# Rongjiehuang/FastDiff

Hardware: AMD Instinct MI355X
Metric: real-time factor (audio-sec/wall-sec), N=4 reverse steps, 80x864 mel (higher is better)
Workload: dtype f32 results; 2-piece fp16 operands (22 bit) on fp16 MFMA, fp32 accumulate; GEMM as Winograd F(2,3); exact-fp32 twin; 1 GPU; BASELINE configs[1]: LJSpeech shape, batch=8 x 80x864 mel per GPU, N=4, HIP kernels + hipGraph sampler; batch_per_gpu=8, frames=864, reverse_steps=4, graph=True, weights=random init seed 1234 (no checkpoint offline), world_size=1, gpus_visible=1, oversubscribed=False

## Files before the change

fastdiff_amd/csrc/fd_kernels_lvc.hip:

```cpp
#include "fd_kernels_common.h"

namespace fdk_fast {

template <int HOP, int DIL>
struct LvcCfg {
    static constexpr int WC = 64;
    static constexpr int W = 4 * WC;
    static constexpr int H = (DIL + 1 + 3) & ~3;
    static constexpr int XLD = W + 2 * H;
    static constexpr int YLD = W + 4;
};

#ifdef FD_LVC_TIMING
__device__ long long fd_dbg[64 * 4 * 8];
#define FD_STAMP(i) do { if (lane == 0 && blockIdx.y == FD_LVC_TIMING && blockIdx.x >= 100 && blockIdx.x < 164) \
        fd_dbg[((blockIdx.x - 100) * 4 + wave) * 8 + (i)] = (long long)__builtin_amdgcn_s_memtime(); } while (0)
#elif defined(FD_LVC_TIMELINE)
__device__ long long *fd_tl;
#define FD_STAMP_AT(i) do { if (threadIdx.x == 0) { long long *q_ = fd_tl + ((size_t)blockIdx.y * gridDim.x + blockIdx.x) * 10; \
        q_[i] = (long long)__builtin_amdgcn_s_memrealtime(); \
        if ((i) == 0) { q_[8] = __builtin_amdgcn_s_getreg(63492); q_[9] = __builtin_amdgcn_s_getreg(63508); } } } while (0)
#if defined(FD_TL_VARIANT)
#define FD_STAMP(i) do { if ((i) == 0 || (i) == 6 || (i) == 7) FD_STAMP_AT(i); else if ((i) == 1) FD_STAMP_AT(5); } while (0)
#define FD_STAMP_X(i) FD_STAMP_AT(i)
#else
#define FD_STAMP(i) FD_STAMP_AT(i)
#endif
#else
#define FD_STAMP(i)
#endif
#ifndef FD_STAMP_X
#define FD_STAMP_X(i)
#endif

__device__ __forceinline__ float gate(float a, float b)
{
    typedef float f2 __attribute__((ext_vector_type(2)));
    b = fmaxf(b, -15.0f);
    const f2 e = f2{a, b} * f2{-1.4426950408889634f, -2.8853900817779268f};
    const f2 uv = f2{__builtin_amdgcn_exp2f(e.x), __builtin_amdgcn_exp2f(e.y)};
    const f2 d = uv + 1.0f;
    return (1.0f - uv.y) * __builtin_amdgcn_rcpf(d.x * d.y);
}

template <int HOP, int DIL>
__global__ void __launch_bounds__(256, 2) k_lvc_layer(const float *__restrict__ xin, const float *__restrict__ skip,
                                                      float *__restrict__ xout, const float *__restrict__ kpack, int layer,
                                                      const float *__restrict__ wpack, const float *__restrict__ wref,
                                                      const float *__restrict__ cbias, int T, const int *__restrict__ run_if,
                                                      const int *__restrict__ lens)
{
    static_assert(HOP >= 64, "hop 8 has its own kernel (k_lvc_h8)");
    using Cfg = LvcCfg<HOP, DIL>;
    if (run_if && *run_if == 0) return;
    constexpr int WC = Cfg::WC, W = Cfg::W, H = Cfg::H, XLD = Cfg::XLD, YLD = Cfg::YLD, NT = WC / 32;
    constexpr int LT = (HOP == 256) ? 1 : 2;
    constexpr int LN = (HOP == 256) ? 4 : 2;
    constexpr bool PREACT = (HOP == 256);
    __shared__ __attribute__((aligned(16))) float xs[fd::C * XLD];
    __shared__ __attribute__((aligned(16))) float ys[fd::C * YLD];
    const int Ln = T * HOP;
    const int b = blockIdx.y, w0 = blockIdx.x * W;
    const int Tb = frames_of(lens, b, T), Lnb = Tb * HOP;
    if (w0 >= Lnb) return;
    const int tid = threadIdx.x, lane = tid & 63, wave = tid >> 6, l31 = lane & 31, hi = lane >> 5;
    const int cw = wave * WC;
    const bool wave_valid = (w0 + cw) < Lnb;
    const int mt0 = (HOP == 256) ? (wave & 1) : 0;
    const int lcw = (HOP == 256) ? 128 * (wave >> 1) : cw;
    FD_STAMP(0);

    float4 ka[LT][12];
    float4 bz[LT][4];
    if constexpr (HOP >= 64) {
        if (wave_valid) {
            const int f = (w0 + lcw) / HOP;
            const float *rec = kpack + ((int64_t)b * T + f) * fd::KREC;
            const float4 *kp4 = reinterpret_cast<const float4 *>(rec + layer * fd::KLAYER) + 2 * lane;
            const float4 *kb4 = reinterpret_cast<const float4 *>(rec + fd::KW + layer * 64);
#pragma unroll
            for (int m = 0; m < LT; ++m) {
#pragma unroll
                for (int i = 0; i < 12; ++i) ka[m][i] = kp4[((mt0 + m) * 6 + (i >> 1)) * 128 + (i & 1)];
#pragma unroll
                for (int j = 0; j < 4; ++j) bz[m][j] = kb4[(mt0 + m) * 8 + 2 * j + hi];
            }
        }
    }
    float4 wa[12];
#pragma unroll
    for (int i = 0; i < 12; ++i) wa[i] = reinterpret_cast<const float4 *>(wpack)[i * 64 + lane];
    float4 cb[4];
#pragma unroll
    for (int j = 0; j < 4; ++j) cb[j] = reinterpret_cast<const float4 *>(cbias)[2 * j + hi];
    {
        const float *xr = xin + (int64_t)b * fd::C * Ln, *sr = skip + (int64_t)b * fd::C * Ln;
        constexpr int NF4 = XLD / 4, TOTAL = fd::C * NF4, NK = (TOTAL + 255) / 256;
        constexpr int NB = (HOP == 64) ? 2 : 1, KB = (NK + NB - 1) / NB;
#pragma unroll
        for (int bt = 0; bt < NB; ++bt) {
            float4 xa[KB], sa[KB];
#pragma unroll
            for (int k = 0; k < KB; ++k) {
                const int idx = (bt * KB + k) * 256 + tid, ci = idx / NF4, c4 = idx - ci * NF4, g = w0 - H + 4 * c4;
                const bool ok = idx < TOTAL && g >= 0 && g < Lnb;
                xa[k] = ok ? *reinterpret_cast<const float4 *>(xr + (int64_t)ci * Ln + g) : make_float4(0.f, 0.f, 0.f, 0.f);
                sa[k] = ok ? *reinterpret_cast<const float4 *>(sr + (int64_t)ci * Ln + g) : make_float4(0.f, 0.f, 0.f, 0.f);
            }
            __builtin_amdgcn_sched_barrier(0);
#pragma unroll
            for (int k = 0; k < KB; ++k) {
                const int idx = (bt * KB + k) * 256 + tid, ci = idx / NF4, c4 = idx - ci * NF4;
                if (idx < TOTAL) {
                    const float4 r = make_float4(xa[k].x + sa[k].x, xa[k].y + sa[k].y, xa[k].z + sa[k].z, xa[k].w + sa[k].w);
                    if constexpr (PREACT) {
                        *reinterpret_cast<float4 *>(xs + ci * XLD + 4 * c4) =
                            make_float4(lrelu(r.x, 0.2f), lrelu(r.y, 0.2f), lrelu(r.z, 0.2f), lrelu(r.w, 0.2f));
                        if (c4 >= H / 4 && c4 < H / 4 + W / 4) *reinterpret_cast<float4 *>(ys + ci * YLD + 4 * c4 - H) = r;
                    } else {
                        *reinterpret_cast<float4 *>(xs + ci * XLD + 4 * c4) = r;
                    }
                }
            }
        }
    }
    const int hside = tid >> 7, ho = (tid & 127) >> 2, hq = tid & 3;
    __syncthreads();
    FD_STAMP(1);
    float resid[PREACT ? LN : 1][PREACT ? 8 * LT : 1];
    if constexpr (PREACT) {
#pragma unroll
        for (int nt = 0; nt < LN; ++nt)
#pragma unroll
            for (int m = 0; m < LT; ++m)
#pragma unroll
                for (int r = 0; r < 8; ++r)
                    resid[nt][m * 8 + r] = ys[(16 * (mt0 + m) + (r & 3) + 8 * (r >> 2) + 4 * hi) * YLD + lcw + nt * 32 + l31];
        __syncthreads();
    }

    if (wave_valid) {
        f32x16 acc[NT];
#pragma unroll
        for (int ct = 0; ct < NT; ++ct) {
#pragma unroll
            for (int r = 0; r < 16; ++r) acc[ct][r] = f4c(cb[r >> 2], r & 3);
            const int col = hi * XLD + H + cw + ct * 32 + l31;
            const int o[3] = {opaque(col - DIL), opaque(col), opaque(col + DIL)};
#pragma unroll
            for (int s = 0; s < 48; ++s) {
                const int tap = s >> 4, c2 = (2 * s) & 31;
                const float xv = xs[o[tap] + c2 * XLD];
                const float v = PREACT ? xv : lrelu(xv, 0.2f);
                acc[ct] = mfma32(f4c(wa[s >> 2], s & 3), v, acc[ct]);
                if (ct > 0 && s % 3 == 1) {
                    const int r = s / 3, cp = cw + (ct - 1) * 32 + l31;
                    ys[drow(r, hi) * YLD + cp + 1] = (w0 + cp) < Lnb ? lrelu(acc[ct - 1][r], 0.2f) : 0.0f;
                }
            }
        }
        {
            const int cp = cw + (NT - 1) * 32 + l31;
            const bool inside = (w0 + cp) < Lnb;
#pragma unroll
            for (int r = 0; r < 16; ++r) ys[drow(r, hi) * YLD + cp + 1] = inside ? lrelu(acc[NT - 1][r], 0.2f) : 0.0f;
        }
    } else {
#pragma unroll
        for (int ct = 0; ct < NT; ++ct)
#pragma unroll
            for (int r = 0; r < 16; ++r) ys[drow(r, hi) * YLD + cw + ct * 32 + l31 + 1] = 0.0f;
    }
    FD_STAMP(2);
    {
        float4 hwt[6];
#pragma unroll
        for (int j = 0; j < 6; ++j) hwt[j] = reinterpret_cast<const float4 *>(wref + (ho * fd::C + 8 * hq) * 3)[j];
        const float hbias = cbias[ho];
        const int c = hside ? W : -1, g = w0 + c;
        float accv = 0.0f;
        if (g >= 0 && g < Lnb) {
            const float wv[24] = {hwt[0].x, hwt[0].y, hwt[0].z, hwt[0].w, hwt[1].x, hwt[1].y, hwt[1].z, hwt[1].w,
                                  hwt[2].x, hwt[2].y, hwt[2].z, hwt[2].w, hwt[3].x, hwt[3].y, hwt[3].z, hwt[3].w,
                                  hwt[4].x, hwt[4].y, hwt[4].z, hwt[4].w, hwt[5].x, hwt[5].y, hwt[5].z, hwt[5].w};
#pragma unroll
            for (int j = 0; j < 8; ++j)
#pragma unroll
                for (int tap = 0; tap < 3; ++tap)
                {
                    const float xv = xs[(8 * hq + j) * XLD + H + c + (tap - 1) * DIL];
                    accv += wv[j * 3 + tap] * (PREACT ? xv : lrelu(xv, 0.2f));
                }
        }
        accv += __shfl_xor(accv, 1, 64);
        accv += __shfl_xor(accv, 2, 64);
        if (hq == 0) ys[ho * YLD + c + 1] = (g >= 0 && g < Lnb) ? lrelu(accv + hbias, 0.2f) : 0.0f;
    }
    FD_STAMP(3);
    __syncthreads();
    FD_STAMP(4);
    if (!wave_valid) return;

    const int64_t orow = (int64_t)b * fd::C * Ln;
    if constexpr (HOP >= 64) {
        float *xo = xout + orow + (int64_t)(4 * hi) * Ln + w0 + lcw + l31;
        const unsigned Lnu = (unsigned)Ln;
        f32x16 a[LN][LT];
        auto epilogue_row = [&](int nt, int m, int r) {
            const int chl = 16 * (mt0 + m) + (r & 3) + 8 * (r >> 2);
            float xr;
            if constexpr (PREACT) xr = resid[nt][m * 8 + r];
            else xr = xs[(chl + 4 * hi) * XLD + H + lcw + nt * 32 + l31];
            xo[(unsigned)chl * Lnu + (unsigned)(nt * 32)] = xr + gate(a[nt][m][r], a[nt][m][r + 8]);
        };
        constexpr int EPI = 8 * LT, GAP = 48 / EPI;
#pragma unroll
        for (int nt = 0; nt < LN; ++nt) {
#pragma unroll
            for (int m = 0; m < LT; ++m)
#pragma unroll
                for (int r = 0; r < 16; ++r) a[nt][m][r] = f4c(bz[m][r >> 2], r & 3);
            const int yc = hi * 8 * YLD + lcw + nt * 32 + l31;
            const int yo[3] = {opaque(yc), opaque(yc + 1), opaque(yc + 2)};
#pragma unroll
            for (int s = 0; s < 48; ++s) {
                const int tap = s >> 4, c2 = 16 * ((s >> 3) & 1) + (s & 7);
                const float v = ys[yo[tap] + c2 * YLD];
#pragma unroll
                for (int m = 0; m < LT; ++m) a[nt][m] = mfma32(f4c(ka[m][s >> 2], s & 3), v, a[nt][m]);
                if (nt > 0 && s % GAP == GAP / 2) {
                    const int e = s / GAP;
                    epilogue_row(nt - 1, e / 8, e % 8);
                }
            }
            if (nt == 0) FD_STAMP(5);
        }
        FD_STAMP(6);
#pragma unroll
        for (int e = 0; e < EPI; ++e) epilogue_row(LN - 1, e / 8, e % 8);
        FD_STAMP(7);
    }
}

template <int HOP, int DIL, bool FINAL, int UP = 0>
__global__ void __launch_bounds__(256, 2) k_lvc_h2(const float *__restrict__ xin, const float *__restrict__ skip, float *__restrict__ xout,
                                                   const float *__restrict__ kpack, int layer, const float4 *__restrict__ wpack16,
                                                   const float *__restrict__ wref, const float *__restrict__ cbias,
                                                   int *__restrict__ range_flag, int T, const int *__restrict__ lens,
                                                   float *__restrict__ eps_acc, const float4 *__restrict__ ffuse,
                                                   const float4 *__restrict__ up_pack16, const float *__restrict__ up_bias,
                                                   int *__restrict__ up_flag)
{
    static_assert(!FINAL || HOP == 256, "the fused final conv relies on whole-tile utterance lengths");
    static_assert(UP == 0 || (DIL == 1 && (UP == 4 || UP == 8)), "the fused up-sampler belongs to the first layer of a block");
    constexpr int W = 256, WC = 64, H = (DIL + 1 + 3) & ~3, XC = W + 2 * H, YC = W + 2;
    constexpr int UPPAD = UP ? UP : 1, UPN = UP ? (W + 2 * UPPAD) / UPPAD : 0, UPROWS = UPN + 2;
    __shared__ __attribute__((aligned(16))) char xp_img[UP ? UPROWS * 128 : 16];
    __shared__ float hsk[UP ? fd::C * 2 * H : 1];
    constexpr int LT = (HOP == 256) ? 1 : 2;
    constexpr int LN = (HOP == 256) ? 4 : 2;
    static_assert(2 * H <= 64, "one halo column per lane");
    __shared__ __attribute__((aligned(16))) char xs[XC * 128];
    __shared__ __attribute__((aligned(16))) char ys[YC * 128];
    static_assert(YC * 128 >= fd::C * W * 4, "parking area");
    const int Ln = T * HOP;
    const int ntile = (T * HOP + W - 1) / W, tile = lvc_tile_of_workgroup();
    const int b = blockIdx.y, w0 = tile * W;
    const int Lnb = frames_of(lens, b, T) * HOP;
    if (tile >= ntile || w0 >= Lnb || skip_after_previous_overflow(range_flag)) return;
    const int tid = threadIdx.x, lane = tid & 63, wave = tid >> 6, l31 = lane & 31, hi = lane >> 5;
    const int cw = wave * WC;
    const bool wave_valid = (w0 + cw) < Lnb;
    const int mt0 = (HOP == 256) ? (wave & 1) : 0;
    const int lcw = (HOP == 256) ? 128 * (wave >> 1) : cw;
    float mx = 0.0f;
    FD_STAMP(0);

    float4 ka[LT][12];
    float4 bz[LT][4];
    auto load_kernel = [&](int m) {
        if (HOP == 256 || wave_valid) {
            const int f = (w0 + lcw) / HOP;
            const float *rec = kpack + ((int64_t)b * T + f) * fd::KREC;
            const float4 *kp4 = reinterpret_cast<const float4 *>(rec + layer * fd::KLAYER) + 2 * lane;
            const float4 *kb4 = reinterpret_cast<const float4 *>(rec + fd::KW + layer * 64);
#pragma unroll
            for (int i = 0; i < 12; ++i) ka[m][i] = lvc_ld<4>(kp4 + ((mt0 + m) * 6 + (i >> 1)) * 128 + (i & 1));
#pragma unroll
            for (int j = 0; j < 4; ++j) bz[m][j] = kb4[(mt0 + m) * 8 + 2 * j + hi];
        }
    };
    __shared__ float4 ffs[FINAL ? 64 : 1];
    if constexpr (FINAL) {
        if (tid < 64) ffs[tid] = ffuse[tid];
    }
#ifndef FD_LVC_LATE_KERNEL
    if constexpr (HOP == 256) load_kernel(0);
#endif
    float4 wa[2][6];
    float4 cb[4];
    float hbias;
    auto load_conv_weights = [&]() {
#pragma unroll
        for (int p = 0; p < 2; ++p)
#pragma unroll
            for (int kg = 0; kg < 6; ++kg) wa[p][kg] = wpack16[(p * 6 + kg) * 64 + lane];
#pragma unroll
        for (int j = 0; j < 4; ++j) cb[j] = reinterpret_cast<const float4 *>(cbias)[2 * j + hi];
        hbias = cbias[l31];
    };
    if constexpr (UP == 0) load_conv_weights();
#ifdef FD_LVC_PAD_LOADS
    {
        float4 pad_[FD_LVC_PAD_LOADS];
#pragma unroll
        for (int i_ = 0; i_ < FD_LVC_PAD_LOADS; ++i_) pad_[i_] = wpack16[(i_ % 12) * 64 + lane];
#pragma unroll
        for (int i_ = 0; i_ < FD_LVC_PAD_LOADS; ++i_) mx = fmaxf(mx, fminf(pad_[i_].x, 0.0f) * 1e-30f);
    }
#endif

    {
        const float *xr = xin + ((int64_t)b * fd::C + wave * 8) * Ln, *sr = skip + ((int64_t)b * fd::C + wave * 8) * Ln;
        const int g = w0 + 4 * lane;
        const bool ok = g < Lnb;
        const int hc = lane, hg = (hc < H) ? w0 - H + hc : w0 + W + hc - H;
        const bool hok = hc < 2 * H && hg >= 0 && hg < Lnb;
        float4 xa[8], sa[8];
        float hx[8], hs[8];
#pragma unroll
        for (int c = 0; c < 8; ++c) {
#ifdef FD_LVC_PROBE_NOLOADX
            const float pv_ = __int_as_float(0x3c000000 | (lane << 8) | (c << 4));
            if constexpr (UP == 0) xa[c] = make_float4(pv_, -pv_, pv_ * 0.5f, pv_ * 0.25f);
            sa[c] = make_float4(pv_ * 0.125f, pv_, -pv_, pv_ * 2.0f);
#else
            if constexpr (UP == 0) xa[c] = ok ? lvc_ld<1>(reinterpret_cast<const float4 *>(xr + (int64_t)c * Ln + g)) : make_float4(0.f, 0.f, 0.f, 0.f);
            sa[c] = ok ? lvc_ld<8>(reinterpret_cast<const float4 *>(sr + (int64_t)c * Ln + g)) : make_float4(0.f, 0.f, 0.f, 0.f);
#endif
        }
#pragma unroll
        for (int c = 0; c < 8; ++c) {
#ifdef FD_LVC_PROBE_NOLOADX
            if constexpr (UP == 0) hx[c] = __int_as_float(0x3b000000 | (lane << 8) | (c << 4));
            hs[c] = hok ? 0.03125f : 0.0f;
#else
            if constexpr (UP == 0) hx[c] = hok ? xr[(int64_t)c * Ln + hg] : 0.0f;
            hs[c] = hok ? sr[(int64_t)c * Ln + hg] : 0.0f;
#endif
        }
#ifdef FD_LVC_PROBE_UP_NOCONVT
        if constexpr (UP > 0) {
            load_conv_weights();
#pragma unroll
            for (int c = 0; c < 8; ++c) {
                const float pv_ = __int_as_float(0x3c000000 | (lane << 8) | (c << 4));
                xa[c] = make_float4(pv_, -pv_, pv_ * 0.5f, pv_ * 0.25f);
                hx[c] = pv_ * 0.125f;
            }
            (void)xp_img; (void)hsk; (void)up_pack16; (void)up_bias;
        }
#else
        if constexpr (UP > 0) {
            constexpr int R = UP, NT = (UPN + 31) / 32, PHW = R / 4;
            const int Lq = Ln / R, Lqb = Lnb / R, q0 = w0 / R;
            {
                constexpr int NU = 4 * UPROWS, NK = (NU + 255) / 256;
                float v[NK][8];
#pragma unroll
                for (int k = 0; k < NK; ++k) {
                    const int u = k * 256 + tid, cg = u / UPROWS, jj = u - cg * UPROWS, j = q0 - 2 + jj;
                    const bool okp = u < NU && j >= 0 && j < Lqb;
#pragma unroll
                    for (int c = 0; c < 8; ++c) v[k][c] = okp ? xin[((int64_t)b * fd::C + cg * 8 + c) * Lq + j] : 0.0f;
                }
#pragma unroll
                for (int k = 0; k < NK; ++k) {
                    const int u = k * 256 + tid, cg = u / UPROWS, jj = u - cg * UPROWS;
                    if (u < NU) {
#pragma unroll
                        for (int c = 0; c < 8; ++c) { mx = fmaxf(mx, fabsf(v[k][c])); v[k][c] = lrelu(v[k][c], 0.2f); }
                        float4 ph, pl;
                        split8(v[k], ph, pl);
                        *reinterpret_cast<float4 *>(xp_img + h2_off(jj, cg)) = ph;
                        *reinterpret_cast<float4 *>(xp_img + h2_off(jj, 4 + cg)) = pl;
                    }
                }
            }
            float4 ub[4];
#pragma unroll
            for (int j = 0; j < 4; ++j) ub[j] = reinterpret_cast<const float4 *>(up_bias)[2 * j + hi];
            float4 wun[2][4];
#pragma unroll
            for (int p = 0; p < 2; ++p)
#pragma unroll
                for (int kg = 0; kg < 4; ++kg) wun[p][kg] = up_pack16[(((wave * PHW) * 2 + p) * 4 + kg) * 64 + lane];
            __syncthreads();
            FD_STAMP_X(1);
            float *park = reinterpret_cast<float *>(ys);
#pragma unroll
            for (int pw = 0; pw < PHW; ++pw) {
                const int ph = wave * PHW + pw;
                float4 wu[2][4];
#pragma unroll
                for (int p = 0; p < 2; ++p)
#pragma unroll
                    for (int kg = 0; kg < 4; ++kg) wu[p][kg] = wun[p][kg];
                if (pw + 1 < PHW) {
#pragma unroll
                    for (int p = 0; p < 2; ++p)
#pragma unroll
                        for (int kg = 0; kg < 4; ++kg) wun[p][kg] = up_pack16[(((ph + 1) * 2 + p) * 4 + kg) * 64 + lane];
                }
                const int offA = (ph < R / 2) ? 0 : 1, offB = offA - 1;
#pragma unroll
                for (int t = 0; t < NT; ++t) {
                    const int ql = 32 * t + l31, qc = min(ql, UPN - 1);
                    f32x16 ah, al;
#pragma unroll
                    for (int r = 0; r < 16; ++r) { ah[r] = f4c(ub[r >> 2], r & 3); al[r] = 0.0f; }
#pragma unroll
                    for (int kg = 0; kg < 4; ++kg) {
                        const int row = qc + 1 + ((kg >> 1) ? offB : offA), c2 = kg & 1;
                        const float4 b1 = *reinterpret_cast<const float4 *>(xp_img + h2_off(row, c2 * 2 + hi));
                        const float4 b2 = *reinterpret_cast<const float4 *>(xp_img + h2_off(row, 4 + c2 * 2 + hi));
                        ah = mfma_f16(wu[0][kg], b1, ah);
                        al = mfma_f16(wu[0][kg], b2, al);
                        al = mfma_f16(wu[1][kg], b1, al);
                    }
                    const int col = R * ql + ph - UPPAD;
                    if (ql < UPN && col >= -H && col < W + H) {
                        const int gc = w0 + col;
                        const bool inb = gc >= 0 && gc < Lnb;
                        const int pcol = ph * (W / R) + ((ql - 1) ^ ((R == 8) ? 16 * (ph >> 2) : 0));
                        float *dst = (col >= 0 && col < W) ? park + pcol : hsk + (col < 0 ? col + H : col - W + H);
                        const int cs = (col >= 0 && col < W) ? W : 2 * H;
#pragma unroll
                        for (int r = 0; r < 16; ++r)
                            dst[(8 * (r >> 2) + 4 * hi + (r & 3)) * cs] = inb ? fmaf(al[r], GX_INV_SCALE, ah[r]) : 0.0f;
                    }
                }
            }
            FD_STAMP_X(2);
            __syncthreads();
            FD_STAMP_X(3);
            load_conv_weights();
            {
                const float *pk = reinterpret_cast<const float *>(ys) + wave * 8 * W +
                                  (R == 4 ? lane : (4 * (lane & 1)) * (W / R) + ((lane >> 1) ^ (16 * (lane & 1))));
#pragma unroll
                for (int c = 0; c < 8; ++c)
                    xa[c] = make_float4(pk[c * W], pk[c * W + (W / R)], pk[c * W + 2 * (W / R)], pk[c * W + 3 * (W / R)]);
            }
#pragma unroll
            for (int c = 0; c < 8; ++c) hx[c] = hc < 2 * H ? hsk[(wave * 8 + c) * (2 * H) + hc] : 0.0f;
            FD_STAMP_X(4);
        }
#endif
#ifdef FD_LVC_LATE_KERNEL
        __builtin_amdgcn_sched_barrier(0);
        if constexpr (HOP == 256 && UP == 0) load_kernel(0);
#endif
        __builtin_amdgcn_sched_barrier(0);
#pragma unroll
        for (int c = 0; c < 8; ++c) {
            xa[c] = make_float4(xa[c].x + sa[c].x, xa[c].y + sa[c].y, xa[c].z + sa[c].z, xa[c].w + sa[c].w);
            mx = amax4(mx, xa[c]);
            *reinterpret_cast<float4 *>(ys + ((wave * 8 + c) * W + 4 * lane) * 4) = xa[c];
        }
#pragma unroll
        for (int j = 0; j < 4; ++j) {
            float v[8];
#pragma unroll
            for (int c = 0; c < 8; ++c) v[c] = lrelu(f4c(xa[c], j), 0.2f);
            float4 ph, pl;
            split8(v, ph, pl);
            const int row = H + 4 * lane + j;
            *reinterpret_cast<float4 *>(xs + h2_off(row, wave)) = ph;
            *reinterpret_cast<float4 *>(xs + h2_off(row, 4 + wave)) = pl;
        }
        if (hc < 2 * H) {
            float v[8];
#pragma unroll
            for (int c = 0; c < 8; ++c) {
                const float t = hx[c] + hs[c];
                mx = fmaxf(mx, fabsf(t));
                v[c] = lrelu(t, 0.2f);
            }
            float4 ph, pl;
            split8(v, ph, pl);
            const int row = (hc < H) ? hc : W + hc;
            *reinterpret_cast<float4 *>(xs + h2_off(row, wave)) = ph;
            *reinterpret_cast<float4 *>(xs + h2_off(row, 4 + wave)) = pl;
        }
    }
    if constexpr (HOP != 256) load_kernel(0);
    __syncthreads();
    FD_STAMP(1);
    float resid[LN][8 * LT];
    {
#pragma unroll
        for (int nt = 0; nt < LN; ++nt)
#pragma unroll
            for (int m = 0; m < LT; ++m)
#pragma unroll
                for (int r = 0; r < 8; ++r)
                    resid[nt][m * 8 + r] =
                        reinterpret_cast<const float *>(ys)[(16 * (mt0 + m) + (r & 3) + 8 * (r >> 2) + 4 * hi) * W + lcw + nt * 32 + l31];
        __syncthreads();
    }
    FD_STAMP(2);

    if (wave_valid) {
        int xo_[3][2][2];
#pragma unroll
        for (int tap = 0; tap < 3; ++tap) {
            const int row = H + cw + l31 + (tap - 1) * DIL;
#pragma unroll
            for (int p = 0; p < 2; ++p)
#pragma unroll
                for (int c2 = 0; c2 < 2; ++c2) xo_[tap][p][c2] = h2_off(row, p * 4 + c2 * 2 + hi);
        }
#pragma unroll
        for (int ct = 0; ct < 2; ++ct) {
            f32x16 ah, al;
#pragma unroll
            for (int r = 0; r < 16; ++r) { ah[r] = f4c(cb[r >> 2], r & 3); al[r] = 0.0f; }
#pragma unroll
            for (int kg = 0; kg < 6; ++kg) {
                const float4 b1 = *reinterpret_cast<const float4 *>(xs + xo_[kg >> 1][0][kg & 1] + ct * 32 * 128);
                const float4 b2 = *reinterpret_cast<const float4 *>(xs + xo_[kg >> 1][1][kg & 1] + ct * 32 * 128);
                ah = mfma_f16(wa[0][kg], b1, ah);
                al = mfma_f16(wa[0][kg], b2, al);
                al = mfma_f16(wa[1][kg], b1, al);
            }
            const int cp = cw + ct * 32 + l31, yrow = cp + 1;
            const bool inside = (w0 + cp) < Lnb;
#pragma unroll
            for (int j = 0; j < 4; ++j) {
                float v[4];
#pragma unroll
                for (int i = 0; i < 4; ++i) {
                    v[i] = inside ? lrelu(fmaf(al[4 * j + i], GX_INV_SCALE, ah[4 * j + i]), 0.2f) : 0.0f;
                    mx = fmaxf(mx, fabsf(v[i]));
                }
                uint2 ph, pl;
                split2(v[0], v[1], ph.x, pl.x);
                split2(v[2], v[3], ph.y, pl.y);
                *reinterpret_cast<uint2 *>(ys + h2_off(yrow, j) + 8 * hi) = ph;
                *reinterpret_cast<uint2 *>(ys + h2_off(yrow, 4 + j) + 8 * hi) = pl;
            }
        }
    } else {
#pragma unroll
        for (int s8 = 0; s8 < 8; ++s8) *reinterpret_cast<float4 *>(ys + (cw + 1 + lane) * 128 + s8 * 16) = make_float4(0.f, 0.f, 0.f, 0.f);
    }
    if constexpr (HOP != 256) load_kernel(1);
    FD_STAMP(3);
    if (wave < 2) {
        const int c = wave ? W : -1, g = w0 + c;
        const bool ok = g >= 0 && g < Lnb;
        float a1 = 0.0f, a2 = 0.0f;
        if (ok) {
#pragma unroll
            for (int kg = 0; kg < 6; ++kg) halo_dot(xs, H + c + ((kg >> 1) - 1) * DIL, (kg & 1) * 2 + hi, wa[0][kg], wa[1][kg], a1, a2);
        }
        float accv = fmaf(a2, GX_INV_SCALE, a1);
        accv += __shfl_xor(accv, 32, 64);
        if (hi == 0) {
            const float v = ok ? lrelu(accv + hbias, 0.2f) : 0.0f;
            mx = fmaxf(mx, fabsf(v));
            const _Float16 v1 = (_Float16)v, v2 = (_Float16)((v - (float)v1) * GX_SCALE);
            const int yrow = c + 1;
            *reinterpret_cast<_Float16 *>(ys + h2_off(yrow, l31 >> 3) + (l31 & 7) * 2) = v1;
            *reinterpret_cast<_Float16 *>(ys + h2_off(yrow, 4 + (l31 >> 3)) + (l31 & 7) * 2) = v2;
        }
    }
    FD_STAMP(4);
    __syncthreads();
    FD_STAMP(5);
    if (wave_valid) {
        float4 kh[LT][6], kl[LT][6];
#pragma unroll
        for (int m = 0; m < LT; ++m)
#pragma unroll
            for (int kg = 0; kg < 6; ++kg) {
                const float4 &a0 = ka[m][2 * kg], &a1 = ka[m][2 * kg + 1];
                mx = amax4(amax4(mx, a0), a1);
                const float v[8] = {a0.x, a0.y, a0.z, a0.w, a1.x, a1.y, a1.z, a1.w};
                split8(v, kh[m][kg], kl[m][kg]);
            }
        int yo_[3][2][2];
#pragma unroll
        for (int tap = 0; tap < 3; ++tap) {
            const int row = lcw + l31 + tap;
#pragma unroll
            for (int p = 0; p < 2; ++p)
#pragma unroll
                for (int c2 = 0; c2 < 2; ++c2) yo_[tap][p][c2] = h2_off(row, p * 4 + c2 * 2 + hi);
        }
        const int64_t ooff = (int64_t)b * fd::C * Ln + (int64_t)(4 * hi) * Ln + w0 + lcw + l31;
        float *xo = xout + ooff;
        FD_STAMP(6);
#ifdef FD_LVC_PAD_VALU
        {
            float pad_ = mx;
#pragma unroll
            for (int i_ = 0; i_ < FD_LVC_PAD_VALU; ++i_) asm volatile("v_fma_f32 %0, %0, %0, %0" : "+v"(pad_));
            mx = fminf(mx, pad_ * 0.0f + mx);
        }
#endif
        const unsigned Lnu = (unsigned)Ln;
#pragma unroll
        for (int nt = 0; nt < LN; ++nt) {
#pragma unroll
            for (int m = 0; m < LT; ++m) {
                f32x16 ah, al;
#pragma unroll
                for (int r = 0; r < 16; ++r) { ah[r] = f4c(bz[m][r >> 2], r & 3); al[r] = 0.0f; }
#pragma unroll
                for (int kg = 0; kg < 6; ++kg) {
                    const float4 b1 = *reinterpret_cast<const float4 *>(ys + yo_[kg >> 1][0][kg & 1] + nt * 32 * 128);
                    const float4 b2 = *reinterpret_cast<const float4 *>(ys + yo_[kg >> 1][1][kg & 1] + nt * 32 * 128);
                    ah = mfma_f16(kh[m][kg], b1, ah);
                    al = mfma_f16(kh[m][kg], b2, al);
                    al = mfma_f16(kl[m][kg], b1, al);
                }
#pragma unroll
                for (int r = 0; r < 8; ++r) {
                    const int chl = 16 * (mt0 + m) + (r & 3) + 8 * (r >> 2);
                    const float zs = fmaf(al[r], GX_INV_SCALE, ah[r]), zt = fmaf(al[r + 8], GX_INV_SCALE, ah[r + 8]);
                    if constexpr (FINAL) resid[nt][m * 8 + r] += gate(zs, zt);
#ifdef FD_LVC_PROBE_NOSTORE
                    else { const float keep_ = resid[nt][m * 8 + r] + gate(zs, zt); asm volatile("" :: "v"(keep_)); (void)xo; (void)Lnu; (void)chl; }
#else
                    else lvc_st<2>(xo + ((unsigned)chl * Lnu + (unsigned)(nt * 32)), resid[nt][m * 8 + r] + gate(zs, zt));
#endif
                }
            }
        }
    }
#ifdef FD_LVC_PROBE_FINAL_NOFOLD
    if constexpr (FINAL) {
#pragma unroll
        for (int nt = 0; nt < LN; ++nt)
#pragma unroll
            for (int r = 0; r < 8; ++r) asm volatile("" :: "v"(resid[nt][r]));
        (void)eps_acc; (void)ffs;
    }
#else
    if constexpr (FINAL) {
        FD_STAMP_X(1);
        float *pb = reinterpret_cast<float *>(xs);
        {
            const int part = 2 * mt0 + hi;
            float fw[8][8];
#pragma unroll
            for (int r = 0; r < 8; ++r) {
                const float4 lo4 = ffs[(part * 8 + r) * 2], hi4 = ffs[(part * 8 + r) * 2 + 1];
                fw[r][0] = lo4.x; fw[r][1] = lo4.y; fw[r][2] = lo4.z; fw[r][3] = lo4.w; fw[r][4] = hi4.x; fw[r][5] = hi4.y; fw[r][6] = hi4.z;
            }
#pragma unroll
            for (int nt = 0; nt < LN; ++nt)
#pragma unroll
                for (int k = 0; k < 7; ++k) {
                    float pk = 0.0f;
#pragma unroll
                    for (int r = 0; r < 8; ++r) pk = fmaf(fw[r][k], resid[nt][r], pk);
                    pb[(part * 7 + k) * W + lcw + nt * 32 + l31] = pk;
                }
        }
        FD_STAMP_X(2);
        __syncthreads();
        FD_STAMP_X(3);
        auto column_sum = [&](int t) {
            float e = 0.0f;
#pragma unroll
            for (int k = 0; k < 7; ++k) {
                const int col = t + k - 3;
                if (col >= 0 && col < W) {
#pragma unroll
                    for (int part = 0; part < 4; ++part) e += pb[(part * 7 + k) * W + col];
                }
            }
            return e;
        };
        float *ea = eps_acc + (int64_t)b * Ln + w0;
        const float e = column_sum(tid);
        if (tid >= 3 && tid < W - 3) ea[tid] = e;
        else atomicAdd(ea + tid, e);
        if (tid >= 64 && tid < 70) {
            const int j = tid - 64, t = j < 3 ? j - 3 : W + j - 3;
            if (w0 + t >= 0 && w0 + t < Lnb) atomicAdd(ea + t, column_sum(t));
        }
        FD_STAMP_X(4);
    }
#endif
    if (!(mx < GX_LIMIT)) {
        atomicOr(range_flag, 1);
        if constexpr (UP > 0) atomicOr(up_flag, 1);
    }
    FD_STAMP(7);
}
template <int DIL>
__global__ void __launch_bounds__(256, 2) k_lvc_h8(const float *__restrict__ xin, const float *__restrict__ skip, float *__restrict__ xout,
                                                   const float *__restrict__ kpack, int layer, const float *__restrict__ wref,
                                                   const float *__restrict__ cbias, int T, const int *__restrict__ lens,
                                                   const int *__restrict__ run_if)
{
    constexpr int HOP = 8, W = 32, H = (DIL + 1 + 3) & ~3, XLD = W + 2 * H, YLD = 12;
    if (run_if && *run_if == 0) return;
    __shared__ __attribute__((aligned(16))) float xs[fd::C * XLD];
    __shared__ __attribute__((aligned(16))) float xr[fd::C * W];
    __shared__ __attribute__((aligned(16))) float ys[4][fd::C * YLD];
    __shared__ float wl[fd::C * 3 * fd::C];
    const int Ln = T * HOP;
    const int b = blockIdx.y, w0 = blockIdx.x * W;
    const int Tb = frames_of(lens, b, T), Lnb = Tb * HOP;
    if (w0 >= Lnb) return;
    const int tid = threadIdx.x, lane = tid & 63, wave = tid >> 6, l31 = lane & 31, hi = lane >> 5;
    const int f = w0 / HOP + wave;
    const bool frame_valid = f < Tb;
    float4 ke[12], ko[12];
    float bzv = 0.0f;
    if (frame_valid) {
        const float *rec = kpack + ((int64_t)b * T + f) * fd::KREC;
        const float4 *kp4 = reinterpret_cast<const float4 *>(rec + layer * fd::KLAYER) + (hi * 6 * 64 + l31) * 2;
#pragma unroll
        for (int i = 0; i < 12; ++i) { ke[i] = kp4[(i >> 1) * 128 + (i & 1)]; ko[i] = kp4[(i >> 1) * 128 + 64 + (i & 1)]; }
        bzv = rec[fd::KW + layer * 64 + lane];
    }
    float wst[12];
#pragma unroll
    for (int k = 0; k < 12; ++k) { const int idx = k * 256 + tid; wst[k] = wref[(idx & 31) * (fd::C * 3) + (idx >> 5)]; }
    const float cbv = cbias[l31];
    {
        const float *xp = xin + (int64_t)b * fd::C * Ln, *sp = skip + (int64_t)b * fd::C * Ln;
        constexpr int NF4 = XLD / 4, TOTAL = fd::C * NF4, NK = (TOTAL + 255) / 256;
        float4 xa[NK], sa[NK];
#pragma unroll
        for (int k = 0; k < NK; ++k) {
            const int idx = k * 256 + tid, ci = idx / NF4, c4 = idx - ci * NF4, g = w0 - H + 4 * c4;
            const bool ok = idx < TOTAL && g >= 0 && g < Lnb;
            xa[k] = ok ? *reinterpret_cast<const float4 *>(xp + (int64_t)ci * Ln + g) : make_float4(0.f, 0.f, 0.f, 0.f);
            sa[k] = ok ? *reinterpret_cast<const float4 *>(sp + (int64_t)ci * Ln + g) : make_float4(0.f, 0.f, 0.f, 0.f);
        }
#pragma unroll
        for (int k = 0; k < NK; ++k) {
            const int idx = k * 256 + tid, ci = idx / NF4, c4 = idx - ci * NF4;
            if (idx < TOTAL) {
                const float4 r = make_float4(xa[k].x + sa[k].x, xa[k].y + sa[k].y, xa[k].z + sa[k].z, xa[k].w + sa[k].w);
                *reinterpret_cast<float4 *>(xs + ci * XLD + 4 * c4) = make_float4(lrelu(r.x, 0.2f), lrelu(r.y, 0.2f), lrelu(r.z, 0.2f), lrelu(r.w, 0.2f));
                if (c4 >= H / 4 && c4 < H / 4 + W / 4) *reinterpret_cast<float4 *>(xr + ci * W + 4 * c4 - H) = r;
            }
        }
    }
#pragma unroll
    for (int k = 0; k < 12; ++k) wl[k * 256 + tid] = wst[k];
    __syncthreads();
    if (!frame_valid) return;
    {
        float acc[5] = {cbv, cbv, cbv, cbv, cbv};
        const float *xb = xs + H + 8 * wave - 1 + 5 * hi;
#pragma unroll 2
        for (int in = 0; in < fd::C; ++in)
#pragma unroll
            for (int k = 0; k < 3; ++k) {
                const float wv = wl[(in * 3 + k) * fd::C + l31];
                const float *xq = xb + in * XLD + (k - 1) * DIL;
#pragma unroll
                for (int c = 0; c < 5; ++c) acc[c] = fmaf(wv, xq[c], acc[c]);
            }
#pragma unroll
        for (int c = 0; c < 5; ++c) {
            const int g = w0 + 8 * wave - 1 + 5 * hi + c;
            ys[wave][l31 * YLD + 5 * hi + c] = (g >= 0 && g < Lnb) ? lrelu(acc[c], 0.2f) : 0.0f;
        }
    }
    __builtin_amdgcn_fence(__ATOMIC_RELEASE, "wavefront");
    __builtin_amdgcn_wave_barrier();
    float z[8];
#pragma unroll
    for (int c = 0; c < 8; ++c) z[c] = bzv;
#pragma unroll
    for (int in = 0; in < fd::C; ++in) {
        const float *yr = ys[wave] + in * YLD;
        const float4 y0 = *reinterpret_cast<const float4 *>(yr);
        const float4 y1 = *reinterpret_cast<const float4 *>(yr + 4);
        const float2 y2 = *reinterpret_cast<const float2 *>(yr + 8);
        const float yv[10] = {y0.x, y0.y, y0.z, y0.w, y1.x, y1.y, y1.z, y1.w, y2.x, y2.y};
#pragma unroll
        for (int tap = 0; tap < 3; ++tap) {
            const int kk = tap * 32 + in, kg = kk >> 4, e = kk & 7;
            const float kv = (kk & 8) ? f4c(ko[2 * kg + (e >> 2)], e & 3) : f4c(ke[2 * kg + (e >> 2)], e & 3);
#pragma unroll
            for (int c = 0; c < 8; ++c) z[c] = fmaf(kv, yv[c + tap], z[c]);
// ... 301 lines not shown
```

Measured before the change: 10030 x real-time.

## Compute UP=4 upsampler output directly in registers, skipping shared-memory parking

For the UP=4 fused up-sampler layer, each wave now computes its transposed-conv MFMA tiles straight into the register layout the LVC input stage expects. This removes the park-to-shared-memory pass, the extra barrier and the halo staging buffer. Threads are remapped (sg/sl) so each wave owns a channel group and time half, and halo columns are computed by a separate small MFMA tile. Conv weights and kernel bias loads are deferred until after this work. The cost is more per-wave MFMA work and register pressure, plus a more intricate lane mapping that could be wrong at edges.

```diff
diff --git a/fastdiff_amd/csrc/fd_kernels_lvc.hip b/fastdiff_amd/csrc/fd_kernels_lvc.hip
--- a/fastdiff_amd/csrc/fd_kernels_lvc.hip
+++ b/fastdiff_amd/csrc/fd_kernels_lvc.hip
@@ -254,9 +254,14 @@
     static_assert(!FINAL || HOP == 256, "the fused final conv relies on whole-tile utterance lengths");
     static_assert(UP == 0 || (DIL == 1 && (UP == 4 || UP == 8)), "the fused up-sampler belongs to the first layer of a block");
     constexpr int W = 256, WC = 64, H = (DIL + 1 + 3) & ~3, XC = W + 2 * H, YC = W + 2;
+#ifdef FD_LVC_PROBE_UP_NOCONVT
+    constexpr bool UP4 = false;
+#else
+    constexpr bool UP4 = (UP == 4);
+#endif
     constexpr int UPPAD = UP ? UP : 1, UPN = UP ? (W + 2 * UPPAD) / UPPAD : 0, UPROWS = UPN + 2;
     __shared__ __attribute__((aligned(16))) char xp_img[UP ? UPROWS * 128 : 16];
-    __shared__ float hsk[UP ? fd::C * 2 * H : 1];
+    __shared__ float hsk[UP == 8 ? fd::C * 2 * H : 1];
     constexpr int LT = (HOP == 256) ? 1 : 2;
     constexpr int LN = (HOP == 256) ? 4 : 2;
     static_assert(2 * H <= 64, "one halo column per lane");
@@ -278,16 +283,20 @@
 
     float4 ka[LT][12];
     float4 bz[LT][4];
-    auto load_kernel = [&](int m) {
+    auto load_kernel = [&](int m, bool kernel = true, bool bias = true) {
         if (HOP == 256 || wave_valid) {
             const int f = (w0 + lcw) / HOP;
             const float *rec = kpack + ((int64_t)b * T + f) * fd::KREC;
             const float4 *kp4 = reinterpret_cast<const float4 *>(rec + layer * fd::KLAYER) + 2 * lane;
             const float4 *kb4 = reinterpret_cast<const float4 *>(rec + fd::KW + layer * 64);
-#pragma unroll
-            for (int i = 0; i < 12; ++i) ka[m][i] = lvc_ld<4>(kp4 + ((mt0 + m) * 6 + (i >> 1)) * 128 + (i & 1));
-#pragma unroll
-            for (int j = 0; j < 4; ++j) bz[m][j] = kb4[(mt0 + m) * 8 + 2 * j + hi];
+            if (kernel) {
+#pragma unroll
+                for (int i = 0; i < 12; ++i) ka[m][i] = lvc_ld<4>(kp4 + ((mt0 + m) * 6 + (i >> 1)) * 128 + (i & 1));
+            }
+            if (bias) {
+#pragma unroll
+                for (int j = 0; j < 4; ++j) bz[m][j] = kb4[(mt0 + m) * 8 + 2 * j + hi];
+            }
         }
     };
     __shared__ float4 ffs[FINAL ? 64 : 1];
@@ -295,7 +304,7 @@
         if (tid < 64) ffs[tid] = ffuse[tid];
     }
 #ifndef FD_LVC_LATE_KERNEL
-    if constexpr (HOP == 256) load_kernel(0);
+    if constexpr (HOP == 256) load_kernel(0, true, !UP4);
 #endif
     float4 wa[2][6];
     float4 cb[4];
@@ -321,8 +330,9 @@
 #endif
 
     {
-        const float *xr = xin + ((int64_t)b * fd::C + wave * 8) * Ln, *sr = skip + ((int64_t)b * fd::C + wave * 8) * Ln;
-        const int g = w0 + 4 * lane;
+        const int sg = UP4 ? 2 * (wave >> 1) + hi : wave, sl = UP4 ? 32 * (wave & 1) + l31 : lane;
+        const float *xr = xin + ((int64_t)b * fd::C + sg * 8) * Ln, *sr = skip + ((int64_t)b * fd::C + sg * 8) * Ln;
+        const int g = w0 + 4 * sl;
         const bool ok = g < Lnb;
         const int hc = lane, hg = (hc < H) ? w0 - H + hc : w0 + W + hc - H;
         const bool hok = hc < 2 * H && hg >= 0 && hg < Lnb;
@@ -346,9 +356,34 @@
             hs[c] = hok ? 0.03125f : 0.0f;
 #else
             if constexpr (UP == 0) hx[c] = hok ? xr[(int64_t)c * Ln + hg] : 0.0f;
-            hs[c] = hok ? sr[(int64_t)c * Ln + hg] : 0.0f;
-#endif
-        }
+            if constexpr (!UP4) hs[c] = hok ? sr[(int64_t)c * Ln + hg] : 0.0f;
+#endif
+        }
+        const int hcol2 = (l31 == 0 ? -H : W) + 2 * (wave & 1);
+        const bool hok2 = UP4 && l31 < 2 && w0 + hcol2 >= 0 && w0 + hcol2 < Lnb;
+        float2 hs2[UP4 ? 8 : 1];
+        if constexpr (UP4) {
+#pragma unroll
+            for (int c = 0; c < 8; ++c)
+                hs2[c] = hok2 ? *reinterpret_cast<const float2 *>(sr + (int64_t)c * Ln + w0 + hcol2) : make_float2(0.0f, 0.0f);
+        }
+        float4 wu4[2][UP4 ? 4 : 1], ub8[2];
+        [[maybe_unused]] auto up_tile = [&](int row0, int tp, float (&res)[16]) {
+            f32x16 ah, al;
+#pragma unroll
+            for (int r = 0; r < 16; ++r) { ah[r] = f4c(ub8[r >> 3], 2 * ((r >> 2) & 1) + ((r & 3) >> 1)); al[r] = 0.0f; }
+#pragma unroll
+            for (int kg = 0; kg < (UP4 ? 4 : 0); ++kg) {
+                const int row = row0 + tp - (kg >> 1), c2 = kg & 1;
+                const float4 b1 = *reinterpret_cast<const float4 *>(xp_img + h2_off(row, c2 * 2 + hi));
+                const float4 b2 = *reinterpret_cast<const float4 *>(xp_img + h2_off(row, 4 + c2 * 2 + hi));
+                ah = mfma_f16(wu4[0][kg], b1, ah);
+                al = mfma_f16(wu4[0][kg], b2, al);
+                al = mfma_f16(wu4[1][kg], b1, al);
+            }
+#pragma unroll
+            for (int r = 0; r < 16; ++r) res[r] = fmaf(al[r], GX_INV_SCALE, ah[r]);
+        };
 #ifdef FD_LVC_PROBE_UP_NOCONVT
         if constexpr (UP > 0) {
             load_conv_weights();
@@ -387,16 +422,46 @@
                     }
                 }
             }
-            float4 ub[4];
-#pragma unroll
-            for (int j = 0; j < 4; ++j) ub[j] = reinterpret_cast<const float4 *>(up_bias)[2 * j + hi];
-            float4 wun[2][4];
-#pragma unroll
-            for (int p = 0; p < 2; ++p)
-#pragma unroll
-                for (int kg = 0; kg < 4; ++kg) wun[p][kg] = up_pack16[(((wave * PHW) * 2 + p) * 4 + kg) * 64 + lane];
+            float4 ub[UP4 ? 1 : 4];
+            float4 wun[2][UP4 ? 1 : 4];
+            const int chh = wave >> 1, tph = wave & 1;
+            const int wrow = hi * 32 + 16 * chh + 8 * ((l31 >> 2) & 1) + 2 * (l31 >> 3) + ((l31 & 3) >> 1);
+            auto up_weights = [&](int tp) {
+                const int ph = 2 * tp + (l31 & 1);
+#pragma unroll
+                for (int p = 0; p < 2; ++p)
+#pragma unroll
+                    for (int kg = 0; kg < (UP4 ? 4 : 0); ++kg) wu4[p][kg] = up_pack16[((ph * 2 + p) * 4 + kg) * 64 + wrow];
+            };
+            if constexpr (UP4) {
+#pragma unroll
+                for (int j = 0; j < 2; ++j) ub8[j] = reinterpret_cast<const float4 *>(up_bias)[2 * sg + j];
+                up_weights(1 - tph);
+            } else {
+#pragma unroll
+                for (int j = 0; j < 4; ++j) ub[j] = reinterpret_cast<const float4 *>(up_bias)[2 * j + hi];
+#pragma unroll
+                for (int p = 0; p < 2; ++p)
+#pragma unroll
+                    for (int kg = 0; kg < 4; ++kg) wun[p][kg] = up_pack16[(((wave * PHW) * 2 + p) * 4 + kg) * 64 + lane];
+            }
             __syncthreads();
             FD_STAMP_X(1);
+            if constexpr (UP4) {
+                float resa[16], resb[16];
+                up_tile(sl + 2, 1 - tph, resa);
+                __builtin_amdgcn_sched_barrier(0);
+                up_weights(tph);
+                up_tile(sl + 2, tph, resb);
+                FD_STAMP_X(2);
+#pragma unroll
+                for (int c = 0; c < 8; ++c) {
+                    const int r = 4 * (c >> 1) + 2 * (c & 1);
+                    const float4 t = tph ? make_float4(resa[r], resa[r + 1], resb[r], resb[r + 1]) : make_float4(resb[r], resb[r + 1], resa[r], resa[r + 1]);
+                    xa[c] = ok ? t : make_float4(0.f, 0.f, 0.f, 0.f);
+                }
+                FD_STAMP_X(3);
+            } else {
             float *park = reinterpret_cast<float *>(ys);
 #pragma unroll
             for (int pw = 0; pw < PHW; ++pw) {
@@ -455,6 +520,7 @@
 #pragma unroll
             for (int c = 0; c < 8; ++c) hx[c] = hc < 2 * H ? hsk[(wave * 8 + c) * (2 * H) + hc] : 0.0f;
             FD_STAMP_X(4);
+            }
         }
 #endif
 #ifdef FD_LVC_LATE_KERNEL
@@ -466,7 +532,7 @@
         for (int c = 0; c < 8; ++c) {
             xa[c] = make_float4(xa[c].x + sa[c].x, xa[c].y + sa[c].y, xa[c].z + sa[c].z, xa[c].w + sa[c].w);
             mx = amax4(mx, xa[c]);
-            *reinterpret_cast<float4 *>(ys + ((wave * 8 + c) * W + 4 * lane) * 4) = xa[c];
+            *reinterpret_cast<float4 *>(ys + ((sg * 8 + c) * W + 4 * sl) * 4) = xa[c];
         }
 #pragma unroll
         for (int j = 0; j < 4; ++j) {
@@ -475,11 +541,11 @@
             for (int c = 0; c < 8; ++c) v[c] = lrelu(f4c(xa[c], j), 0.2f);
             float4 ph, pl;
             split8(v, ph, pl);
-            const int row = H + 4 * lane + j;
-            *reinterpret_cast<float4 *>(xs + h2_off(row, wave)) = ph;
-            *reinterpret_cast<float4 *>(xs + h2_off(row, 4 + wave)) = pl;
-        }
-        if (hc < 2 * H) {
+            const int row = H + 4 * sl + j;
+            *reinterpret_cast<float4 *>(xs + h2_off(row, sg)) = ph;
+            *reinterpret_cast<float4 *>(xs + h2_off(row, 4 + sg)) = pl;
+        }
+        if (!UP4 && hc < 2 * H) {
             float v[8];
 #pragma unroll
             for (int c = 0; c < 8; ++c) {
@@ -492,6 +558,32 @@
             const int row = (hc < H) ? hc : W + hc;
             *reinterpret_cast<float4 *>(xs + h2_off(row, wave)) = ph;
             *reinterpret_cast<float4 *>(xs + h2_off(row, 4 + wave)) = pl;
+        }
+        if constexpr (UP4) {
+            float resh[16];
+            __builtin_amdgcn_sched_barrier(0);
+            up_tile(l31 == 0 ? 1 : UPN, wave & 1, resh);
+            if (l31 < 2) {
+#pragma unroll
+                for (int e = 0; e < 2; ++e) {
+                    float v[8];
+#pragma unroll
+                    for (int c = 0; c < 8; ++c) {
+                        const float t = (hok2 ? resh[4 * (c >> 1) + 2 * (c & 1) + e] : 0.0f) + (e ? hs2[c].y : hs2[c].x);
+                        mx = fmaxf(mx, fabsf(t));
+                        v[c] = lrelu(t, 0.2f);
+                    }
+                    float4 ph, pl;
+                    split8(v, ph, pl);
+                    const int row = H + hcol2 + e;
+                    *reinterpret_cast<float4 *>(xs + h2_off(row, sg)) = ph;
+                    *reinterpret_cast<float4 *>(xs + h2_off(row, 4 + sg)) = pl;
+                }
+            }
+            __builtin_amdgcn_sched_barrier(0);
+            load_conv_weights();
+            load_kernel(0, false, true);
+            FD_STAMP_X(4);
         }
     }
     if constexpr (HOP != 256) load_kernel(0);
```

Result: no change. 10030 x real-time (-0.0%).
